# rvl-lab-utoronto/video_similarity_search

Hardware: NVIDIA B200
Metric: finch_full_hierarchy_embeddings_per_s (higher is better)
Workload: dtype f16 screen (f32 accumulate) + f32/f64 exact re-rank

## Files before the change

### video_similarity_search_b200/csrc/nn_screen_tc.cu

```cuda
#include <cuda.h>
#include <cuda_fp16.h>
#include <cuda_fp16.h>
#include <math.h>
#include <stdlib.h>
#include <string.h>
#include <math_constants.h>

#include <algorithm>
#include <type_traits>
#include <vector>

#include "common.cuh"

namespace slic {

constexpr int TC_BM = 128, TC_BK = 64, TC_UMMA_K = 16;
constexpr int TC_BN_WIDE = 256, TC_BN_NARROW = 128;
constexpr int TC_ARES_SPS = 2;
constexpr bool TC_NARROW_ARES = false;
constexpr int TC_ROW_UNIT = 256;
constexpr uint32_t TC_A_BYTES = TC_BM * TC_BK * 2;
constexpr int TC_ARES_MAX_SLABS = 8;
constexpr uint32_t TC_BAR_BYTES = 384;
constexpr int TC_UQ_DEPTH = 4;
constexpr int TC_TMEM_COLS = 512;
template <int NCTA, bool ARES, bool TOPK> struct TcCfg {
    static constexpr int BN = (ARES && TC_NARROW_ARES) ? TC_BN_NARROW : TC_BN_WIDE;
    static constexpr int ACCS = TC_TMEM_COLS / BN;
    static constexpr bool GROUPED = BN == TC_BN_NARROW;
    static constexpr uint32_t B_ROWS = BN / NCTA;
    static constexpr uint32_t B_BYTES = B_ROWS * TC_BK * 2;
    static constexpr uint32_t A_RES_BYTES = ARES ? TC_ARES_MAX_SLABS * TC_A_BYTES : 0;
    static constexpr int SPS = NCTA == 2 ? (ARES ? TC_ARES_SPS : 2) : 1;
    static constexpr uint32_t SLAB_BYTES = ARES ? B_BYTES : TC_A_BYTES + B_BYTES;
    static constexpr uint32_t STAGE_BYTES = SPS * SLAB_BYTES;
    static constexpr int STAGES = ARES ? (TOPK ? 64 : 96) * 1024 / (int)STAGE_BYTES : (NCTA == 1 ? 4 : 3);
    static_assert(STAGES >= 2 && STAGES <= 6, "ring depth");
    static constexpr uint32_t OPERAND_BYTES = A_RES_BYTES + STAGES * STAGE_BYTES;
    static constexpr uint32_t SMEM_BYTES = OPERAND_BYTES + TC_BAR_BYTES  + 960  +
                                           (TOPK ? 32768u : 0u) ;
    static constexpr uint32_t SYM_THR_BYTES = 2 * 2 * 128 * 2;
    static constexpr uint32_t SYM_SMEM_BYTES = OPERAND_BYTES + TC_BAR_BYTES + SYM_THR_BYTES + (ARES ? 640u : 960u);
    static constexpr uint32_t CORESIDENT_MAX_BYTES = 233472 - 2 * 1024;
    static_assert(TOPK || SYM_SMEM_BYTES <= CORESIDENT_MAX_BYTES,
                  "symmetric variant leaves no shared memory for a co-resident CTA of the upload stream");
    static_assert(TOPK || SMEM_BYTES <= CORESIDENT_MAX_BYTES,
                  "top-1 variant (gated launches) leaves no shared memory for a co-resident CTA of the upload stream");
    static_assert(SMEM_BYTES <= 232448, "exceeds the 227 KB of shared memory a CTA may use");
    static_assert(!ARES || NCTA == 2, "the A-resident variant exists for CTA pairs only");
};
constexpr int TC_MAX_STAGES = 6;
constexpr int TC_EPI_WARPS = 8;
constexpr int TC_THREADS = 64 + 32 * TC_EPI_WARPS;
constexpr int TC_THREADS_SYM = TC_THREADS + 32;
constexpr float TC_DEFAULT_EPS = 0.001953125f + 0.0009765625f + 0.0000152587890625f;
constexpr int TC_TOPK_MAX = 64;
constexpr int TC_HIST_BINS = 128;
constexpr int TC_HIST_STRIDE = 2 * TC_BM;
constexpr uint32_t TC_TOPK_SMEM = TC_HIST_BINS * TC_HIST_STRIDE;
static_assert(TC_TOPK_SMEM == 32768, "TcCfg::SMEM_BYTES assumes 32 KB of histograms");

struct ScreenParams {
    int64_t nq, n;
    int num_k_slabs;
    int64_t self_offset;
    float eps;
    int cap;
    int splits;
    int tiles_per_split;
    int64_t num_units;
    int* cand_idx;
    float* cand_score;
    int* cand_cnt;
    int* cand_flags;
    int topk;
    float* cand_kth;
    int* cand_tb;
    int l2_prefetch;
    float* dump;
    int* error_flag;
    unsigned long long* trace;
    const int4* unit_table;
    const int* gates;
    unsigned int* best_enc;
// ... 237 lines not shown
    return u;
}
__device__ __forceinline__ uint32_t cluster_ctarank() {
    uint32_t r;
    asm volatile("mov.u32 %0, %%cluster_ctarank;" : "=r"(r));
    return r;
}
__device__ __forceinline__ void cluster_sync_all() {
    asm volatile("barrier.cluster.arrive.release.aligned;" ::: "memory");
    asm volatile("barrier.cluster.wait.acquire.aligned;" ::: "memory");
}
__device__ __forceinline__ void tc_fence_before() { asm volatile("tcgen05.fence::before_thread_sync;" ::: "memory"); }
__device__ __forceinline__ void tc_fence_after() { asm volatile("tcgen05.fence::after_thread_sync;" ::: "memory"); }
__device__ __forceinline__ void umma_f16(uint32_t tmem_d, uint64_t desc_a, uint64_t desc_b, uint32_t idesc,
                                          uint32_t accumulate) {
    asm volatile(
        "{\n\t.reg .pred p;\n\t"
        "setp.ne.b32 p, %4, 0;\n\t"
        "tcgen05.mma.cta_group::1.kind::f16 [%0], %1, %2, %3, p;\n\t}"
        ::"r"(tmem_d), "l"(desc_a), "l"(desc_b), "r"(idesc), "r"(accumulate)
        : "memory");
}
__device__ __forceinline__ void umma_commit(uint32_t bar) {
    asm volatile("tcgen05.commit.cta_group::1.mbarrier::arrive::one.shared::cluster.b64 [%0];" ::"r"(bar) : "memory");
}
__device__ __forceinline__ void umma_f16_pair(uint32_t tmem_d, uint64_t desc_a, uint64_t desc_b, uint32_t idesc,
                                               uint32_t accumulate) {
    asm volatile(
        "{\n\t.reg .pred p;\n\t"
        "setp.ne.b32 p, %4, 0;\n\t"
        "tcgen05.mma.cta_group::2.kind::f16 [%0], %1, %2, %3, p;\n\t}"
        ::"r"(tmem_d), "l"(desc_a), "l"(desc_b), "r"(idesc), "r"(accumulate)
        : "memory");
}
__device__ __forceinline__ void umma_commit_pair(uint32_t bar) {
    asm volatile(
        "tcgen05.commit.cta_group::2.mbarrier::arrive::one.shared::cluster.multicast::cluster.b64 [%0], %1;"
        ::"r"(bar), "h"((uint16_t)3)
        : "memory");
}
#define SLIC_V32_OUT(v)                                                                                              \
    "=r"(v[0]), "=r"(v[1]), "=r"(v[2]), "=r"(v[3]), "=r"(v[4]), "=r"(v[5]), "=r"(v[6]), "=r"(v[7]), "=r"(v[8]),     \
        "=r"(v[9]), "=r"(v[10]), "=r"(v[11]), "=r"(v[12]), "=r"(v[13]), "=r"(v[14]), "=r"(v[15]), "=r"(v[16]),      \
        "=r"(v[17]), "=r"(v[18]), "=r"(v[19]), "=r"(v[20]), "=r"(v[21]), "=r"(v[22]), "=r"(v[23]), "=r"(v[24]),     \
        "=r"(v[25]), "=r"(v[26]), "=r"(v[27]), "=r"(v[28]), "=r"(v[29]), "=r"(v[30]), "=r"(v[31])
#define SLIC_V32_INOUT(v)                                                                                            \
    "+r"(v[0]), "+r"(v[1]), "+r"(v[2]), "+r"(v[3]), "+r"(v[4]), "+r"(v[5]), "+r"(v[6]), "+r"(v[7]), "+r"(v[8]),     \
        "+r"(v[9]), "+r"(v[10]), "+r"(v[11]), "+r"(v[12]), "+r"(v[13]), "+r"(v[14]), "+r"(v[15]), "+r"(v[16]),      \
        "+r"(v[17]), "+r"(v[18]), "+r"(v[19]), "+r"(v[20]), "+r"(v[21]), "+r"(v[22]), "+r"(v[23]), "+r"(v[24]),     \
        "+r"(v[25]), "+r"(v[26]), "+r"(v[27]), "+r"(v[28]), "+r"(v[29]), "+r"(v[30]), "+r"(v[31])
__device__ __forceinline__ void tmem_ld_issue(uint32_t taddr, uint32_t (&v)[32]) {
    asm volatile(
        "tcgen05.ld.sync.aligned.32x32b.x32.b32 "
        "{%0,%1,%2,%3,%4,%5,%6,%7,%8,%9,%10,%11,%12,%13,%14,%15,%16,%17,%18,%19,%20,%21,%22,%23,%24,%25,%26,%27,%28,"
        "%29,%30,%31}, [%32];"
        : SLIC_V32_OUT(v)
        : "r"(taddr)
        : "memory");
}
__device__ __forceinline__ void tmem_ld_wait(uint32_t (&v)[32]) {
    asm volatile("tcgen05.wait::ld.sync.aligned;" : SLIC_V32_INOUT(v)::"memory");
}

__device__ __forceinline__ uint64_t umma_smem_desc(uint32_t smem_addr) {
    uint64_t d = 0;
    d |= (uint64_t)((smem_addr & 0x3FFFFu) >> 4);
// ... 405 lines not shown
            int stage = 0;
            uint32_t phase = 0, a_phase = 0;
            unsigned long long t_wait = 0;
            const bool scheduler = cta_rank == 0;
            const int stride_groups = (int)(gridDim.x / NCTA);
            auto draw = [&]() -> int { return p.queue_on_peer ? atomicAdd_system(p.queue, 1) : atomicAdd(p.queue, 1); };
            int u_next = scheduler ? (p.queue ? draw() : (int)(blockIdx.x / NCTA)) : 0;
            while (true) {
                int u;
                if (scheduler) {
                    u = u_next < p.num_units ? u_next : -1;
                    mbar_wait_cluster(bar_uq_empty + 8u * ring.slot, ring.phase ^ 1u, p.error_flag);
#pragma unroll
                    for (uint32_t r = 0; r < (uint32_t)NCTA; ++r) {
                        st_cluster_u32(peer_smem_addr(uq_val + 4u * ring.slot, r), (uint32_t)u);
                        mbar_arrive_release_cluster(peer_smem_addr(bar_uq_full + 8u * ring.slot, r));
                    }
                    if (++ring.slot == TC_UQ_DEPTH) {
                        ring.slot = 0;
                        ring.phase ^= 1u;
                    }
                    if (u >= 0) u_next = p.queue ? draw() : u_next + stride_groups;
                } else {
                    u = ring_take(ring, false, p.error_flag);
                }
                if (u < 0) break;
                const UnitInfo ui = unit_info(p, u, n_col_tiles);
                const int64_t row_block = ui.row_unit * NCTA + cta_rank;
                if (ui.gate >= 0) gate_wait(p.gates + ui.gate, p.error_flag);
                if constexpr (SYM) {
                    if (ui.coldir && p.sync_counter)
                        counter_wait(p.sync_counter, __ldg(p.sync_targets + ui.gate + 1), p.error_flag);
                }
                if constexpr (ARES) {
                    mbar_wait_traced(bar_a_empty, a_phase ^ 1, p.error_flag, t_wait, tracing);
                    if (cta_rank == 0) mbar_expect_tx(bar_a_full, 2 * (uint32_t)p.num_k_slabs * TC_A_BYTES);
                    for (int ks = 0; ks < p.num_k_slabs; ++ks)
                        tma_load_2d_pair(&tmap_q, smem_base + ks * TC_A_BYTES, bar_a_full, ks * TC_BK,
                                         (int)(row_block * TC_BM));
                    a_phase ^= 1;
                }
                for (int kt = 0; kt < ui.count; ++kt) {
                    const int64_t ct = ui.ct0 + (int64_t)kt * ui.stride;
                    if (p.l2_prefetch > 0 && kt + p.l2_prefetch < ui.count) {
                        const int64_t ctp = ui.ct0 + (int64_t)(kt + p.l2_prefetch) * ui.stride;
                        for (int ks = 0; ks < p.num_k_slabs; ++ks)
                            tma_prefetch_l2_2d(&tmap_x, ks * TC_BK, (int)(ctp * BN + cta_rank * Cfg::B_ROWS));
                    }
                    for (int ks = 0; ks < p.num_k_slabs; ks += Cfg::SPS) {
                        mbar_wait_traced(bar_empty + 8 * stage, phase ^ 1, p.error_flag, t_wait, tracing);
                        const uint32_t a_dst = ring_base + stage * Cfg::STAGE_BYTES;
                        const uint32_t b_dst = ARES ? a_dst : a_dst + TC_A_BYTES;
                        if constexpr (ARES) {
                            const int nsl = min(Cfg::SPS, p.num_k_slabs - ks);
                            if (cta_rank == 0) mbar_expect_tx(bar_full + 8 * stage, 2 * (uint32_t)nsl * Cfg::B_BYTES);
                            for (int j = 0; j < nsl; ++j)
                                tma_load_2d_pair(&tmap_x, b_dst + j * Cfg::SLAB_BYTES, bar_full + 8 * stage, (ks + j) * TC_BK,
                                                 (int)(ct * BN + cta_rank * Cfg::B_ROWS));
                        } else if constexpr (NCTA == 2) {
                            const int nsl = min(Cfg::SPS, p.num_k_slabs - ks);
                            if (cta_rank == 0) mbar_expect_tx(bar_full + 8 * stage, 2 * (uint32_t)nsl * Cfg::SLAB_BYTES);
                            for (int j = 0; j < nsl; ++j) {
                                tma_load_2d_pair(&tmap_q, a_dst + j * Cfg::SLAB_BYTES, bar_full + 8 * stage, (ks + j) * TC_BK,
                                                 (int)(row_block * TC_BM));
                                tma_load_2d_pair(&tmap_x, b_dst + j * Cfg::SLAB_BYTES, bar_full + 8 * stage, (ks + j) * TC_BK,
                                                 (int)(ct * BN + cta_rank * Cfg::B_ROWS));
                            }
                        } else {
                            mbar_expect_tx(bar_full + 8 * stage, Cfg::STAGE_BYTES);
                            tma_load_2d(&tmap_q, a_dst, bar_full + 8 * stage, ks * TC_BK, (int)(row_block * TC_BM));
                            tma_load_2d(&tmap_x, b_dst, bar_full + 8 * stage, ks * TC_BK, (int)(ct * BN));
                        }
                        if (++stage == STAGES) {
                            stage = 0;
                            phase ^= 1;
                        }
                    }
                }
            }
            if (tracing) atomicAdd(p.trace + 0, t_wait);
        }
    } else if (warp == 1) {
        if (lane == 0 && cta_rank == 0) {
            int stage = 0;
            uint32_t phase = 0;
            int acc = 0;
            uint32_t acc_phase = 0, a_phase = 0;
            unsigned long long t_acc = 0, t_smem = 0;
            const long long t_begin = tracing ? clock64() : 0;
            unsigned long long t_ring = 0, n_units = 0;
            while (true) {
                const long long tr0 = tracing ? clock64() : 0;
                const int u = ring_take(ring, false, p.error_flag);
                if (tracing) t_ring += (unsigned long long)(clock64() - tr0);
                if (u < 0) break;
                ++n_units;
                const int n_tiles = unit_info(p, u, n_col_tiles).count;
                if constexpr (ARES) {
                    mbar_wait_traced(bar_a_full, a_phase, p.error_flag, t_smem, tracing);
                    tc_fence_after();
                    a_phase ^= 1;
                }
                for (int kt = 0; kt < n_tiles; ++kt) {
                    mbar_wait_traced(bar_acc_empty + 8 * acc, acc_phase ^ 1, p.error_flag, t_acc, tracing);
                    tc_fence_after();
                    const uint32_t tmem_d = tmem_base + (uint32_t)(acc * BN);
                    for (int ks = 0; ks < p.num_k_slabs; ks += Cfg::SPS) {
                        mbar_wait_traced(bar_full + 8 * stage, phase, p.error_flag, t_smem, tracing);
                        tc_fence_after();
                        const uint32_t st_addr = ring_base + stage * Cfg::STAGE_BYTES;
#pragma unroll
                        for (int j = 0; j < Cfg::SPS; ++j) {
                            if (ks + j < p.num_k_slabs) {
                                const uint32_t sl_addr = st_addr + j * Cfg::SLAB_BYTES;
                                const uint64_t da = umma_smem_desc(ARES ? smem_base + (ks + j) * TC_A_BYTES : sl_addr);
                                const uint64_t db = umma_smem_desc(ARES ? sl_addr : sl_addr + TC_A_BYTES);
#pragma unroll
                                for (int k = 0; k < TC_BK / TC_UMMA_K; ++k) {
                                    if constexpr (NCTA == 2)
                                        umma_f16_pair(tmem_d, da + (uint64_t)(2 * k), db + (uint64_t)(2 * k), tc_idesc(BN, 2),
                                                       (uint32_t)((ks | j | k) != 0));
                                    else
                                        umma_f16(tmem_d, da + (uint64_t)(2 * k), db + (uint64_t)(2 * k), tc_idesc(BN, 1),
                                                  (uint32_t)((ks | j | k) != 0));
                                }
                            }
                        }
                        if constexpr (NCTA == 2) umma_commit_pair(bar_empty + 8 * stage);
                        else umma_commit(bar_empty + 8 * stage);
                        if (++stage == STAGES) {
                            stage = 0;
                            phase ^= 1;
                        }
                    }
                    if constexpr (NCTA == 2) umma_commit_pair(bar_acc_full + 8 * acc);
                    else umma_commit(bar_acc_full + 8 * acc);
                    if (++acc == ACCS) {
                        acc = 0;
                        acc_phase ^= 1;
                    }
                }
                if constexpr (ARES) umma_commit_pair(bar_a_empty);
            }
            if (tracing) {
                atomicAdd(p.trace + 1, t_acc);
                atomicAdd(p.trace + 2, t_smem);
                atomicAdd(p.trace + 3, (unsigned long long)(clock64() - t_begin));
                atomicAdd(p.trace + 8, t_ring);
                atomicAdd(p.trace + 10, n_units);
            }
        }
    } else if (SYM && warp == 2 + TC_EPI_WARPS) {
        uint16_t* thr_buf = reinterpret_cast<uint16_t*>(smem + Cfg::OPERAND_BYTES + TC_BAR_BYTES);
        constexpr unsigned ENC_POS_INF = 0xff800000u;
        constexpr int PER_LANE = BN / 32;
        constexpr int DIAG_TILES = TC_ROW_UNIT / BN;
        unsigned tile_seq = 0, cseq0 = 0u, cseq1 = 0u;
        for (int u; (u = ring_take(ring, true, p.error_flag)) >= 0;) {
            const UnitInfo ui = unit_info(p, u, n_col_tiles);
            if (!ui.coldir) {
                tile_seq += (unsigned)ui.count;
                continue;
            }
            if (p.sync_counter) {
                if (lane == 0) counter_wait(p.sync_counter, __ldg(p.sync_targets + ui.gate + 1), p.error_flag);
                __syncwarp();
            }
            for (int kt = 0; kt < ui.count; ++kt, ++tile_seq) {
                const int64_t ct = ui.ct0 + (int64_t)kt * ui.stride;
                if (ct / DIAG_TILES == ui.row_unit) continue;
                const int grp = GROUPED ? (int)(tile_seq & 1u) : 0;
                const unsigned cs = grp ? cseq1 : cseq0;
                const uint32_t buf = cs & 1u, ph = (cs >> 1) & 1u;
                const uint32_t bi = (uint32_t)grp * 2u + buf;
                unsigned e[PER_LANE];
#pragma unroll
                for (int j = 0; j < PER_LANE; ++j) {
                    const int64_t c = ct * BN + lane + 32 * j;
                    e[j] = c < p.n ? __ldcg(p.best_enc + c) : ENC_POS_INF;
                }
                mbar_wait(bar_thr_empty + 8 * bi, ph ^ 1u, p.error_flag);
                const uint32_t ta = smem_u32(thr_buf + (GROUPED ? bi * 128u : buf * 256u)) + 2u * lane;
// ... 72 lines not shown
            } else {
                cx.st.best = -CUDART_INF_F;
                cx.st.thr = -CUDART_INF_F;
            }
            cx.st.cnt = 0;
            cx.st.flags = 0;
            uint32_t va[32], vb[32];
            bool prefetched = false;
            bool first = true;
            for (int kt = 0; kt < ui.count; ++kt, ++seq_all) {
                if (GROUPED && (int)(seq_all & 1u) != half) continue;
                const int acc = (int)(seq_all % (unsigned)ACCS);
                const uint32_t acc_phase = (seq_all / (unsigned)ACCS) & 1u;
                const int64_t ct = ui.ct0 + (int64_t)kt * ui.stride;
                const int64_t col0 = GROUPED ? ct * BN : ct * BN + half * 128;
                bool cdir = false;
                uint32_t thr_tile = 0u;
                uint32_t thr_done_bar = 0u;
                if constexpr (SYM) {
                    cdir = ui.coldir && ct / (TC_ROW_UNIT / BN) != ui.row_unit;
                    if (cdir) {
                        const uint32_t buf = tile_seq & 1u, ph = (tile_seq >> 1) & 1u;
                        const uint32_t bi = GROUPED ? (uint32_t)half * 2u + buf : buf;
                        thr_tile = smem_u32(thr_buf + (GROUPED ? bi : buf * 2 + half) * 128);
                        thr_done_bar = bar_thr_empty + 8 * bi;
                        mbar_wait(bar_thr_full + 8 * bi, ph, p.error_flag);
                        ++tile_seq;
                    }
                }
                if (TOPK || !prefetched) {
                    mbar_wait_traced(bar_acc_full + 8 * acc, acc_phase, p.error_flag, t_full, tracing);
                    tc_fence_after();
                }
                const uint32_t tbase = tmem_base + ((uint32_t)(quad * 32) << 16) + (uint32_t)(acc * BN + (GROUPED ? 0 : half * 128));
                if constexpr (TOPK) {
                    cx.count = !first;
                    if (first) {
#pragma unroll 1
                        for (int c = 0; c < 4; ++c) {
                            tmem_ld_issue(tbase + (uint32_t)(c * 32), va);
                            tmem_ld_wait(va);
                            const int64_t col_base = col0 + c * 32;
                            if (col_base >= p.n || !cx.row_ok) continue;
#pragma unroll
                            for (int t = 0; t < 32; ++t) {
                                if (col_base + t < p.n && col_base + t != cx.self_col)
                                    hist_insert(cx.st, cx.hist, __uint_as_float(va[t]), p.topk);
                            }
                            hist_advance(cx.st, cx.hist, p.topk, p.eps);
                        }
                    }
                }
                const bool plain = col0 + 128 <= p.n && !p.dump &&
                                   (p.self_offset < 0 || row_block * TC_BM + p.self_offset + TC_BM <= col0 ||
                                    row_block * TC_BM + p.self_offset >= col0 + 128);
                if constexpr (TOPK) {
                    tmem_ld_issue(tbase, vb);
#pragma unroll 1
                    for (int c = 0; c < 4; ++c) {
                        tmem_ld_wait(vb);
#pragma unroll
                        for (int t = 0; t < 32; ++t) va[t] = vb[t];
                        if (c < 3) {
                            tmem_ld_issue(tbase + (uint32_t)(32 * (c + 1)), vb);
                        } else {
                            tc_fence_before();
                            __syncwarp();
                            if (lane == 0) {
                                if constexpr (NCTA == 2) mbar_arrive_leader(bar_acc_empty + 8 * acc);
                                else mbar_arrive(bar_acc_empty + 8 * acc);
                            }
                        }
                        epi_chunk<TOPK, false>(cx, va, col0 + 32 * c, plain);
                    }
                } else {
                    if (!prefetched) tmem_ld_issue(tbase, va);
                    prefetched = false;
#pragma unroll 1
                    for (int h = 0; h < 2; ++h) {
                        tmem_ld_wait(va);
                        tmem_ld_issue(tbase + (uint32_t)(64 * h + 32), vb);
                        epi_chunk<false, SYM>(cx, va, col0 + 64 * h, plain, cdir, thr_tile + 128u * h);
                        tmem_ld_wait(vb);
                        if (h == 0) {
                            tmem_ld_issue(tbase + 64u, va);
                        } else {
                            tc_fence_before();
                            __syncwarp();
                            if (lane == 0) {
                                if constexpr (NCTA == 2) mbar_arrive_leader(bar_acc_empty + 8 * acc);
                                else mbar_arrive(bar_acc_empty + 8 * acc);
                            }
                            if (kt + (int)TILE_STEP < ui.count) {
                                const unsigned nxt = seq_all + TILE_STEP;
                                const int acc_n = (int)(nxt % (unsigned)ACCS);
                                const bool ready = __all_sync(0xffffffffu, mbar_test(bar_acc_full + 8 * acc_n, (nxt / (unsigned)ACCS) & 1u));
                                if (ready) {
                                    tc_fence_after();
                                    tmem_ld_issue(tmem_base + ((uint32_t)(quad * 32) << 16) +
                                                      (uint32_t)(acc_n * BN + (GROUPED ? 0 : half * 128)), va);
                                    prefetched = true;
                                }
                            }
                        }
                        epi_chunk<false, SYM>(cx, vb, col0 + 64 * h + 32, plain, cdir, thr_tile + 128u * h + 64u);
                    }
                    if constexpr (SYM) {
                        if (cdir) {
                            __syncwarp();
                            if (lane == 0) mbar_arrive(thr_done_bar);
                        }
                    }
                }
                if constexpr (TOPK) {
                    if (first) pend_flush(cx.pd, cx.st, p.eps, p.cap, p.topk, false, cx.hist, cx.li, cx.ls);
                }
                first = false;
            }
            if constexpr (TOPK) pend_flush(cx.pd, cx.st, p.eps, p.cap, p.topk, true, cx.hist, cx.li, cx.ls);
            if constexpr (SYM) {
                if (cx.row_ok && cx.st.best > -CUDART_INF_F) {
                    const unsigned e = enc_score(cx.st.best);
                    atomicMax(p.best_enc + cx.row, e);
                    if (!ui.coldir)
                        for (int g = 0; g < p.num_peers; ++g) atomicMax(p.peer_best[g] + cx.row, e);
                }
                if (!ui.coldir && p.sync_counter) {
                    if (p.num_peers) __threadfence_system();
                    else __threadfence();
                    __syncwarp();
                    if (lane == 0) {
                        atomicAdd(p.sync_counter, 1);
// ... 271 lines not shown
        return SLIC_ERR_CUDA;
    }
    return SLIC_OK;
}

static bool g_profile = false, g_have_sample = false;
static unsigned long long* g_trace = nullptr;
static cudaEvent_t g_ev_start = nullptr, g_ev_stop = nullptr;
static double g_last_flop = 0.0, g_last_exec_flop = 0.0;

struct ScreenPlan {
    int splits, tiles_per_split;
    int64_t units;
};

static int screen_ncta() {
    static int cached = 0;
    if (cached == 0) {
        const char* e = getenv("SLIC_SCREEN_NCTA");
        cached = (e && atoi(e) == 1) ? 1 : 2;
    }
    return cached;
}

static bool screen_ares_allowed() {
    static int cached = -1;
    if (cached < 0) {
        const char* e = getenv("SLIC_SCREEN_ARES");
        cached = (e && atoi(e) == 0) ? 0 : 1;
    }
    return cached != 0;
}

static int screen_bn(int d_pad) {
    return (TC_NARROW_ARES && screen_ncta() == 2 && d_pad / TC_BK <= TC_ARES_MAX_SLABS && screen_ares_allowed()) ? TC_BN_NARROW
                                                                                                                  : TC_BN_WIDE;
}

static ScreenPlan plan_screen(int64_t nq, int64_t n, int bn) {
    const int ncta = screen_ncta();
    const int64_t row_blocks = ceil_div(nq, TC_BM * ncta), col_tiles = ceil_div(n, bn);
    const int64_t sms = num_sms() / ncta;
    int64_t want = ceil_div(6 * sms, row_blocks);
    const int64_t min_tiles = 8 * (TC_BN_WIDE / bn);
    int64_t max_splits = col_tiles / min_tiles > 0 ? col_tiles / min_tiles : 1;
    int64_t splits = want < 1 ? 1 : (want > max_splits ? max_splits : want);
    ScreenPlan pl;
    pl.tiles_per_split = (int)ceil_div(col_tiles, splits);
    pl.splits = (int)ceil_div(col_tiles, pl.tiles_per_split);
    pl.units = row_blocks * pl.splits;
    return pl;
}

static ScreenPlan plan_screen_topk(int64_t nq, int64_t n, int k, int bn) {
    const int ncta = screen_ncta();
    const int64_t row_blocks = ceil_div(nq, TC_BM * ncta), col_tiles = ceil_div(n, bn);
    const int64_t sms = num_sms() / ncta;
    const int64_t startup = 6 * (TC_BN_WIDE / bn);
    int64_t best_s = 1, best_cost = INT64_MAX;
    const int64_t min_tps = ceil_div((int64_t)32 * k, bn / 2);
    for (int pass = 0; pass < 2; ++pass) {
        for (int64_t sp = 1; sp <= col_tiles && sp <= 64; ++sp) {
            const int64_t tps = ceil_div(col_tiles, sp);
            if (sp > 1 && tps < min_tps) break;
            const int64_t real = ceil_div(col_tiles, tps);
            const int64_t waves = ceil_div(row_blocks * real, sms);
            const int64_t cost = waves * (tps + startup);
            if (pass == 0) {
                if (cost < best_cost) {
// ... 43 lines not shown
}

static int* g_timeout_record_host = nullptr;
static int arm_timeout_record() {
    if (!g_timeout_record_host) {
        SLIC_CUDA_OK(cudaHostAlloc(&g_timeout_record_host, 8 * sizeof(int), cudaHostAllocMapped));
        int* dev_view = nullptr;
        SLIC_CUDA_OK(cudaHostGetDevicePointer(&dev_view, g_timeout_record_host, 0));
        SLIC_CUDA_OK(cudaMemcpyToSymbol(g_timeout_record, &dev_view, sizeof(dev_view)));
    }
    for (int i = 0; i < 8; ++i) g_timeout_record_host[i] = 0;
    return SLIC_OK;
}
const char* timeout_record_text() {
    static thread_local char buf[160];
    const int* r = g_timeout_record_host;
    if (!r || r[0] == 0) return "";
    snprintf(buf, sizeof(buf), " [timed-out wait: site %d (1 mbarrier, 2 upload gate, 3 pre-pass counter) block %d thread %d a=%d b=%d]",
             r[0], r[1], r[2], r[3], r[4]);
    return buf;
}

static int launch_screen(const uint16_t* q_f16, int64_t nq, const uint16_t* x_f16, int64_t n, int d_pad,
                         int64_t self_offset, float eps, int cap, const ScreenPlan& pl, int* cand_idx, float* cand_score,
                         int* cand_cnt, int* cand_flags, float* dump, int* error_flag, cudaStream_t st, int topk = 0,
                         float* cand_kth = nullptr, const int4* unit_table = nullptr, const int* gates = nullptr,
                         unsigned int* best_enc = nullptr, int64_t exec_tiles = 0, int* log_q = nullptr,
                         int log_region = 0, int* sync_counter = nullptr, const int* sync_targets = nullptr,
                         const ScreenPeers* peers = nullptr, int* cand_tb = nullptr, int* shared_queue = nullptr) {
    const int ncta = screen_ncta();
    if (gates) SLIC_PROPAGATE(arm_timeout_record());
    CUtensorMap tq, tx;
    SLIC_PROPAGATE(make_tmap(&tq, q_f16, nq, d_pad, TC_BM));
    const int bn = screen_bn(d_pad);
    SLIC_PROPAGATE(make_tmap(&tx, x_f16, n, d_pad, bn / ncta));
    ScreenParams p;
    p.nq = nq;
    p.n = n;
    p.num_k_slabs = d_pad / TC_BK;
    p.self_offset = self_offset;
    p.eps = eps;
    p.cap = cap;
    p.splits = pl.splits;
    p.tiles_per_split = pl.tiles_per_split;
    p.num_units = pl.units;
    p.cand_idx = cand_idx;
    p.cand_score = cand_score;
    p.cand_cnt = cand_cnt;
    p.cand_flags = cand_flags;
    p.topk = topk;
    p.cand_kth = cand_kth;
    p.cand_tb = cand_tb;
    {
        static int l2pf = -1;
        if (l2pf < 0) {
            const char* e = getenv("SLIC_SCREEN_L2PF");
            l2pf = e ? atoi(e) : 0;
            if (l2pf < 0 || l2pf > 16) l2pf = 0;
        }
        p.l2_prefetch = l2pf;
    }
    p.dump = dump;
    p.error_flag = error_flag;
    p.trace = g_trace;
    p.unit_table = unit_table;
    p.gates = gates;
    p.best_enc = best_enc;
// ... 235 lines not shown
                if (need != gate) continue;
                const int64_t ct0 = (int64_t)s * pl->tiles_per_split;
                int64_t cnt = ceil_div(n, bn) - ct0;
                if (cnt > pl->tiles_per_split) cnt = pl->tiles_per_split;
                table->push_back(unit_entry(r, ct0, (int)cnt, 1, gate, s, false));
            }
    SLIC_REQUIRE((int64_t)table->size() == pl->units, "gated screen: internal unit count mismatch");
    return SLIC_OK;
}

template <typename T>
static int nn_top1_sym_impl(const T* unit, const uint16_t* ub, int64_t n, int d, int d_pad, float eps, int* idx_out,
                            T* dist_out, int* stats_out, cudaStream_t st, int part, int parts, const GateSpec* gate,
                            AfterScreenFn after, void* after_ctx, bool* overflowed, int mode = 0,
                            const int* bests_in = nullptr, int* bests_out = nullptr, int* stats_ext = nullptr,
                            const ScreenPeers* peers = nullptr, AfterScreenFn before_screen = nullptr,
                            void* before_ctx = nullptr);
static bool screen_sym_allowed();
constexpr int64_t SYM_MIN_ROWS_FWD = 16384;

template <typename T>
static int nn_top1_impl(const T* q_unit, const uint16_t* q_f16, int64_t nq, const T* x_unit, const uint16_t* x_f16,
                        int64_t n, int d, int d_pad, int64_t self_offset, float eps, int* idx_out, T* dist_out,
                        int* stats_out, cudaStream_t st, const GateSpec* gate = nullptr, AfterScreenFn after = nullptr,
                        void* after_ctx = nullptr, int* stats_ext = nullptr) {
    if (q_f16 == x_f16 && q_unit == x_unit && nq == n && self_offset == 0 && n >= SYM_MIN_ROWS_FWD && screen_sym_allowed()) {
        bool overflowed = false;
        SLIC_PROPAGATE(nn_top1_sym_impl<T>(x_unit, x_f16, n, d, d_pad, eps, idx_out, dist_out, stats_out, st, 0, 1, gate,
                                           after, after_ctx, &overflowed, 0, nullptr, nullptr, stats_ext));
        if (stats_ext || !overflowed) return SLIC_OK;
        gate = nullptr;
        after = nullptr;
    }
    ScreenPlan pl = plan_screen(nq, n, screen_bn(d_pad));
    std::vector<int4> table;
    Scratch table_dev;
    if (gate) {
        SLIC_PROPAGATE(plan_screen_gated(nq, n, screen_bn(d_pad), self_offset, *gate, &pl, &table));
        SLIC_CUDA_OK(table_dev.alloc(table.size() * sizeof(int4), st));
        SLIC_PROPAGATE(stage_to_device(table_dev.ptr, table.data(), table.size() * sizeof(int4), st));
    }
    const int64_t slots = (int64_t)pl.splits * 2 * nq;
    Scratch ci, cs, cc, cf, ovr, stats;
    SLIC_CUDA_OK(ci.alloc(slots * TC_CAP * sizeof(int), st));
    SLIC_CUDA_OK(cs.alloc(slots * TC_CAP * sizeof(float), st));
    SLIC_CUDA_OK(cc.alloc(slots * sizeof(int), st));
    SLIC_CUDA_OK(cf.alloc(slots * sizeof(int), st));
    SLIC_CUDA_OK(ovr.alloc(nq * sizeof(int), st));
    int* stats_dev = stats_ext;
    if (!stats_dev) {
        SLIC_CUDA_OK(stats.alloc(8 * sizeof(int), st));
        stats_dev = stats.as<int>();
    }
    SLIC_CUDA_OK(cudaMemsetAsync(stats_dev, 0, 8 * sizeof(int), st));
    SLIC_PROPAGATE(launch_screen(q_f16, nq, x_f16, n, d_pad, self_offset, eps, TC_CAP, pl, ci.as<int>(), cs.as<float>(),
                                 cc.as<int>(), cf.as<int>(), nullptr, stats_dev + 4, st, 0, nullptr,
                                 gate ? table_dev.as<int4>() : nullptr, gate ? gate->gates : nullptr));
    if (after) SLIC_PROPAGATE(after(after_ctx));
    rerank_top1_kernel<T><<<(unsigned)ceil_div(nq, 8), 256, 0, st>>>(q_unit, x_unit, nq, d, eps, TC_CAP, 2 * pl.splits,
                                                                     ci.as<int>(), cs.as<float>(), cc.as<int>(),
                                                                     cf.as<int>(), idx_out, dist_out, ovr.as<int>(),
                                                                     stats_dev);
    SLIC_LAUNCH_OK();
    if (stats_ext) return SLIC_OK;
    int host_stats[8];
    SLIC_CUDA_OK(cudaMemcpyAsync(host_stats, stats_dev, sizeof(host_stats), cudaMemcpyDeviceToHost, st));
    SLIC_CUDA_OK(cudaStreamSynchronize(st));
    if (host_stats[4] != 0) {
        set_error("nn_screen_kernel: pipeline barrier timed out");
        return SLIC_ERR_CUDA;
    }
    const int n_over = host_stats[1];
    if (n_over > 0) {
        Scratch oi, od;
        SLIC_CUDA_OK(oi.alloc((int64_t)n_over * sizeof(int), st));
        SLIC_CUDA_OK(od.alloc((int64_t)n_over * sizeof(T), st));
        SLIC_PROPAGATE(slic_nn_exact_top1(q_unit, ovr.as<int>(), n_over, x_unit, n, d,
                                          sizeof(T) == 4 ? SLIC_F32 : SLIC_F64, self_offset, oi.as<int>(), od.ptr, st));
        scatter_rows_kernel<T><<<(unsigned)ceil_div(n_over, 256), 256, 0, st>>>(ovr.as<int>(), n_over, oi.as<int>(),
                                                                                od.as<T>(), idx_out, dist_out);
        SLIC_LAUNCH_OK();
    }
    if (stats_out) SLIC_CUDA_OK(cudaMemcpyAsync(stats_out, stats_dev, 4 * sizeof(int), cudaMemcpyDeviceToDevice, st));
    return SLIC_OK;
}

template <typename T>
static int topk_tc_impl(const T* q_unit, const uint16_t* q_f16, int64_t nq, const T* x_unit, const uint16_t* x_f16,
                        int64_t n, int d, int d_pad, int k, int64_t self_offset, float eps, int* idx_out, T* dist_out,
                        int* stats_out, cudaStream_t st) {
    const ScreenPlan pl = plan_screen_topk(nq, n, k, screen_bn(d_pad));
    const int TC_CAP_TOPK = topk_cap(k, (int64_t)pl.tiles_per_split * (screen_bn(d_pad) / 2));
    const int64_t slots = (int64_t)pl.splits * 2 * nq;
    Scratch ci, cs, cc, cf, ck, ctb, ovr, stats;
    SLIC_CUDA_OK(ctb.alloc(slots * sizeof(int), st));
    SLIC_CUDA_OK(cudaMemsetAsync(ctb.ptr, 0, slots * sizeof(int), st));
    SLIC_CUDA_OK(ci.alloc(slots * TC_CAP_TOPK * sizeof(int), st));
    SLIC_CUDA_OK(cs.alloc(slots * TC_CAP_TOPK * sizeof(float), st));
    SLIC_CUDA_OK(cc.alloc(slots * sizeof(int), st));
    SLIC_CUDA_OK(cf.alloc(slots * sizeof(int), st));
    SLIC_CUDA_OK(ck.alloc(slots * sizeof(float), st));
    SLIC_CUDA_OK(ovr.alloc(nq * sizeof(int), st));
    SLIC_CUDA_OK(stats.alloc(8 * sizeof(int), st));
    SLIC_CUDA_OK(cudaMemsetAsync(stats.ptr, 0, 8 * sizeof(int), st));
    SLIC_PROPAGATE(launch_screen(q_f16, nq, x_f16, n, d_pad, self_offset, eps, TC_CAP_TOPK, pl, ci.as<int>(),
                                 cs.as<float>(), cc.as<int>(), cf.as<int>(), nullptr, stats.as<int>() + 4, st, k,
                                 ck.as<float>(), nullptr, nullptr, nullptr, 0, nullptr, 0, nullptr, nullptr, nullptr,
                                 ctb.as<int>()));
    rerank_topk_kernel<T><<<(unsigned)nq, RK_THREADS, 0, st>>>(q_unit, x_unit, nq, d, eps, TC_CAP_TOPK, 2 * pl.splits, k,
                                                               ci.as<int>(), cs.as<float>(), cc.as<int>(), cf.as<int>(),
                                                               ck.as<float>(), idx_out, dist_out, ovr.as<int>(),
                                                               stats.as<int>());
    SLIC_LAUNCH_OK();
    int host_stats[8];
    SLIC_CUDA_OK(cudaMemcpyAsync(host_stats, stats.ptr, sizeof(host_stats), cudaMemcpyDeviceToHost, st));
    SLIC_CUDA_OK(cudaStreamSynchronize(st));
    if (host_stats[4] != 0) {
        set_error("nn_screen_kernel: pipeline barrier timed out");
        return SLIC_ERR_CUDA;
    }
    const int n_over = host_stats[1];
    if (n_over > 0) {
        Scratch oi, od;
        SLIC_CUDA_OK(oi.alloc((int64_t)n_over * k * sizeof(int), st));
        SLIC_CUDA_OK(od.alloc((int64_t)n_over * k * sizeof(T), st));
// ... 113 lines not shown
                                                              const typename DistBits<T>::type* __restrict__ row_min,
                                                              const T* __restrict__ edist, int* __restrict__ idx_out,
                                                              T* __restrict__ dist_out) {
    const int64_t base = (int64_t)blockIdx.x * region;
    const int cnt = log_cnt[blockIdx.x];
    for (int e = threadIdx.x; e < cnt; e += blockDim.x) {
        const T dist = edist[base + e];
        if (dist < (T)0) continue;
        const int q = log_q[base + e];
        if (DistBits<T>::of(dist) == row_min[q]) {
            atomicMin(idx_out + q, log_nb[base + e]);
            if (dist_out) dist_out[q] = dist;
        }
    }
}

__global__ void sym_unsettled_rows_kernel(int* __restrict__ idx_out, int64_t n, int* __restrict__ rows, int* __restrict__ stats) {
    const int64_t i = (int64_t)blockIdx.x * blockDim.x + threadIdx.x;
    if (i < n && idx_out[i] == 0x7fffffff) rows[atomicAdd(&stats[1], 1)] = (int)i;
}

template <typename T>
static int nn_top1_sym_impl(const T* unit, const uint16_t* ub, int64_t n, int d, int d_pad, float eps, int* idx_out,
                            T* dist_out, int* stats_out, cudaStream_t st, int part, int parts, const GateSpec* gate,
                            AfterScreenFn after, void* after_ctx, bool* overflowed, int mode, const int* bests_in,
                            int* bests_out, int* stats_ext, const ScreenPeers* peers, AfterScreenFn before_screen,
                            void* before_ctx) {
    typedef typename DistBits<T>::type Bits;
    *overflowed = false;
    ScreenPlan pl;
    std::vector<int4> table;
    int64_t prepass_units_all = 0;
    const bool shared_list = peers && peers->shared_queue;
    SLIC_PROPAGATE(plan_screen_sym(n, screen_bn(d_pad), part, parts, gate, &pl, &table, (SymMode)mode, &prepass_units_all,
                                   shared_list));
    SLIC_REQUIRE((mode == SYM_FUSED) == (peers != nullptr), "symmetric screen: the fused mode needs peer windows (and only it)");
    SLIC_REQUIRE(mode != SYM_FUSED || (stats_ext && !gate), "symmetric screen: the fused mode is asynchronous and ungated");
    int64_t exec_tiles = 0;
    for (const int4& e : table) exec_tiles += e.z & 0xffff;
    const int num_gates = gate ? gate->num_chunks : 0;
    std::vector<int> targets(num_gates + 1, 0);
    for (const int4& e : table) {
        if ((e.w >> 28) & 1) continue;
        const int g = (e.w & 0xfff) - 1;
        for (int k = g + 1; k <= num_gates; ++k) targets[k] += 2 * TC_EPI_WARPS;
    }
    if (mode == SYM_FUSED) targets[0] = (int)(prepass_units_all * 2 * TC_EPI_WARPS);
    const int64_t groups = num_sms() / 2;
    const int64_t grid = (pl.units < groups ? pl.units : groups) * 2;
    const int64_t regions = grid * TC_EPI_WARPS;
    int64_t capacity = (int64_t)SYM_LOG_PER_ROW * n > SYM_LOG_MIN ? (int64_t)SYM_LOG_PER_ROW * n : SYM_LOG_MIN;
    if (mode == SYM_BESTS) capacity = SYM_LOG_MIN;
    const int64_t region = ceil_div(capacity, regions);
    SLIC_REQUIRE(region < ((int64_t)1 << 31), "symmetric screen: log region too large");
    Scratch table_dev, lq, lnb, ls, lcnt, best, rmin, edist, ovr, stats;
    const size_t table_bytes = table.size() * sizeof(int4);
    SLIC_CUDA_OK(table_dev.alloc(table_bytes + (targets.size() + 4) * sizeof(int), st));
    {
        std::vector<unsigned char> blob(table_bytes + (targets.size() + 1) * sizeof(int));
        memcpy(blob.data(), table.data(), table_bytes);
        const int zero = 0;
        memcpy(blob.data() + table_bytes, &zero, sizeof(int));
        memcpy(blob.data() + table_bytes + sizeof(int), targets.data(), targets.size() * sizeof(int));
        SLIC_PROPAGATE(stage_to_device(table_dev.ptr, blob.data(), blob.size(), st));
    }
    int* sync_dev = reinterpret_cast<int*>(static_cast<unsigned char*>(table_dev.ptr) + table_bytes);
    SLIC_CUDA_OK(lq.alloc(regions * region * sizeof(int), st));
// ... 354 lines not shown
        SLIC_CUDA_OK(cudaDeviceSynchronize());
        SLIC_CUDA_OK(cudaFree(g_trace));
        g_trace = nullptr;
    }
    if (g_trace) SLIC_CUDA_OK(cudaMemset(g_trace, 0, 12 * sizeof(uint64_t)));
    return SLIC_OK;
}

int slic_last_screen_time(float* ms_out, double* flop_out) {
    SLIC_REQUIRE(ms_out && flop_out, "last_screen_time: null pointer");
    if (!slic::g_have_sample) {
        slic::set_error("last_screen_time: no profiled launch (call slic_profile_screen(1) first)");
        return SLIC_ERR_INVALID_ARG;
    }
    SLIC_CUDA_OK(cudaEventSynchronize(slic::g_ev_stop));
    SLIC_CUDA_OK(cudaEventElapsedTime(ms_out, slic::g_ev_start, slic::g_ev_stop));
    *flop_out = slic::g_last_flop;
    return SLIC_OK;
}

int slic_last_screen_exec_flop(double* flop_out) {
    SLIC_REQUIRE(flop_out, "last_screen_exec_flop: null pointer");
    *flop_out = slic::g_have_sample ? slic::g_last_exec_flop : 0.0;
    return SLIC_OK;
}

int slic_screen_scores_debug(const uint16_t* q_f16_dev, int64_t nq, const uint16_t* x_f16_dev, int64_t n,
                             int32_t d_pad, float* out_dev, slic_stream_t stream) {
    using namespace slic;
    SLIC_REQUIRE(nq > 0 && n > 0 && d_pad > 0 && d_pad % 64 == 0, "screen_scores_debug: bad shape");
    SLIC_REQUIRE(q_f16_dev && x_f16_dev && out_dev, "screen_scores_debug: null pointer");
    SLIC_PROPAGATE(slic_require_device());
    cudaStream_t st = as_stream(stream);
    const ScreenPlan pl = plan_screen(nq, n, screen_bn(d_pad));
    const int64_t slots = (int64_t)pl.splits * 2 * nq;
    Scratch ci, cs, cc, cf, err;
    SLIC_CUDA_OK(ci.alloc(slots * TC_CAP * sizeof(int), st));
    SLIC_CUDA_OK(cs.alloc(slots * TC_CAP * sizeof(float), st));
    SLIC_CUDA_OK(cc.alloc(slots * sizeof(int), st));
    SLIC_CUDA_OK(cf.alloc(slots * sizeof(int), st));
    SLIC_CUDA_OK(err.alloc(sizeof(int), st));
    SLIC_CUDA_OK(cudaMemsetAsync(err.ptr, 0, sizeof(int), st));
    SLIC_PROPAGATE(launch_screen(q_f16_dev, nq, x_f16_dev, n, d_pad, -1, TC_DEFAULT_EPS, TC_CAP, pl, ci.as<int>(),
                                 cs.as<float>(), cc.as<int>(), cf.as<int>(), out_dev, err.as<int>(), st));
    int host_err = 0;
    SLIC_CUDA_OK(cudaMemcpyAsync(&host_err, err.ptr, sizeof(int), cudaMemcpyDeviceToHost, st));
    SLIC_CUDA_OK(cudaStreamSynchronize(st));
    if (host_err) {
        set_error("nn_screen_kernel: pipeline barrier timed out");
        return SLIC_ERR_CUDA;
    }
    return SLIC_OK;
}

}
```

Measured before the change: 8.793 million.

## Hold resident query operand in tensor memory for non-top-k A-resident screen

For the A-resident, non-top-k CTA-pair screen, the query slabs are now streamed through the shared-memory ring and copied into tensor memory with tcgen05.cp. The MMAs then take A from TMEM and B from shared memory, using a narrower 128-column tile and two accumulators placed after the A columns. This frees the shared memory that previously held the resident A slabs, which goes to a deeper B ring (6 stages, 4 slabs per stage). The cost is a per-unit TMEM copy step and half-width column tiles, which means more tiles and more epilogue passes.

Result: slower. 7.510 million, median of 6 (-14.6%).

```diff
diff --git a/video_similarity_search_b200/csrc/nn_screen_tc.cu b/video_similarity_search_b200/csrc/nn_screen_tc.cu
--- a/video_similarity_search_b200/csrc/nn_screen_tc.cu
+++ b/video_similarity_search_b200/csrc/nn_screen_tc.cu
@@ -17,30 +17,36 @@
 constexpr int TC_BM = 128, TC_BK = 64, TC_UMMA_K = 16;
 constexpr int TC_BN_WIDE = 256, TC_BN_NARROW = 128;
 constexpr int TC_ARES_SPS = 2;
-constexpr bool TC_NARROW_ARES = false;
 constexpr int TC_ROW_UNIT = 256;
 constexpr uint32_t TC_A_BYTES = TC_BM * TC_BK * 2;
 constexpr int TC_ARES_MAX_SLABS = 8;
 constexpr uint32_t TC_BAR_BYTES = 384;
 constexpr int TC_UQ_DEPTH = 4;
 constexpr int TC_TMEM_COLS = 512;
+constexpr uint32_t TC_TMEM_A_COLS = TC_ARES_MAX_SLABS * TC_BK / 2;
+constexpr int TC_MAX_STAGES = 6;
 template <int NCTA, bool ARES, bool TOPK> struct TcCfg {
-    static constexpr int BN = (ARES && TC_NARROW_ARES) ? TC_BN_NARROW : TC_BN_WIDE;
-    static constexpr int ACCS = TC_TMEM_COLS / BN;
-    static constexpr bool GROUPED = BN == TC_BN_NARROW;
+    static constexpr bool TMEM_A = ARES && !TOPK;
+    static constexpr int BN = TMEM_A ? TC_BN_NARROW : TC_BN_WIDE;
+    static constexpr int ACCS = 2;
+    static constexpr uint32_t ACC_COL0 = TMEM_A ? TC_TMEM_A_COLS : 0u;
+    static_assert(ACC_COL0 + ACCS * BN == TC_TMEM_COLS, "TMEM map");
+    static constexpr bool GROUPED = TMEM_A;
     static constexpr uint32_t B_ROWS = BN / NCTA;
     static constexpr uint32_t B_BYTES = B_ROWS * TC_BK * 2;
-    static constexpr uint32_t A_RES_BYTES = ARES ? TC_ARES_MAX_SLABS * TC_A_BYTES : 0;
-    static constexpr int SPS = NCTA == 2 ? (ARES ? TC_ARES_SPS : 2) : 1;
+    static constexpr uint32_t A_RES_BYTES = (ARES && TOPK) ? TC_ARES_MAX_SLABS * TC_A_BYTES : 0;
+    static constexpr int SPS = TMEM_A ? 4 : NCTA == 2 ? (ARES ? TC_ARES_SPS : 2) : 1;
+    static constexpr int A_SPS = 2;
     static constexpr uint32_t SLAB_BYTES = ARES ? B_BYTES : TC_A_BYTES + B_BYTES;
     static constexpr uint32_t STAGE_BYTES = SPS * SLAB_BYTES;
-    static constexpr int STAGES = ARES ? (TOPK ? 64 : 96) * 1024 / (int)STAGE_BYTES : (NCTA == 1 ? 4 : 3);
-    static_assert(STAGES >= 2 && STAGES <= 6, "ring depth");
+    static_assert(!TMEM_A || A_SPS * TC_A_BYTES == STAGE_BYTES, "an A stage fills a ring stage");
+    static constexpr int STAGES = TMEM_A ? TC_MAX_STAGES : ARES ? 64 * 1024 / (int)STAGE_BYTES : (NCTA == 1 ? 4 : 3);
+    static_assert(STAGES >= 2 && STAGES <= TC_MAX_STAGES, "ring depth");
     static constexpr uint32_t OPERAND_BYTES = A_RES_BYTES + STAGES * STAGE_BYTES;
     static constexpr uint32_t SMEM_BYTES = OPERAND_BYTES + TC_BAR_BYTES  + 960  +
                                            (TOPK ? 32768u : 0u) ;
     static constexpr uint32_t SYM_THR_BYTES = 2 * 2 * 128 * 2;
-    static constexpr uint32_t SYM_SMEM_BYTES = OPERAND_BYTES + TC_BAR_BYTES + SYM_THR_BYTES + (ARES ? 640u : 960u);
+    static constexpr uint32_t SYM_SMEM_BYTES = OPERAND_BYTES + TC_BAR_BYTES + SYM_THR_BYTES + 960u;
     static constexpr uint32_t CORESIDENT_MAX_BYTES = 233472 - 2 * 1024;
     static_assert(TOPK || SYM_SMEM_BYTES <= CORESIDENT_MAX_BYTES,
                   "symmetric variant leaves no shared memory for a co-resident CTA of the upload stream");
@@ -49,7 +55,6 @@
     static_assert(SMEM_BYTES <= 232448, "exceeds the 227 KB of shared memory a CTA may use");
     static_assert(!ARES || NCTA == 2, "the A-resident variant exists for CTA pairs only");
 };
-constexpr int TC_MAX_STAGES = 6;
 constexpr int TC_EPI_WARPS = 8;
 constexpr int TC_THREADS = 64 + 32 * TC_EPI_WARPS;
 constexpr int TC_THREADS_SYM = TC_THREADS + 32;
@@ -353,6 +358,18 @@
         "tcgen05.mma.cta_group::2.kind::f16 [%0], %1, %2, %3, p;\n\t}"
         ::"r"(tmem_d), "l"(desc_a), "l"(desc_b), "r"(idesc), "r"(accumulate)
         : "memory");
+}
+__device__ __forceinline__ void umma_f16_pair_ts(uint32_t tmem_d, uint32_t tmem_a, uint64_t desc_b, uint32_t idesc,
+                                                  uint32_t accumulate) {
+    asm volatile(
+        "{\n\t.reg .pred p;\n\t"
+        "setp.ne.b32 p, %4, 0;\n\t"
+        "tcgen05.mma.cta_group::2.kind::f16 [%0], [%1], %2, %3, p;\n\t}"
+        ::"r"(tmem_d), "r"(tmem_a), "l"(desc_b), "r"(idesc), "r"(accumulate)
+        : "memory");
+}
+__device__ __forceinline__ void tmem_cp_pair(uint32_t taddr, uint64_t desc) {
+    asm volatile("tcgen05.cp.cta_group::2.128x256b [%0], %1;" ::"r"(taddr), "l"(desc) : "memory");
 }
 __device__ __forceinline__ void umma_commit_pair(uint32_t bar) {
     asm volatile(
@@ -824,7 +841,21 @@
                     if (ui.coldir && p.sync_counter)
                         counter_wait(p.sync_counter, __ldg(p.sync_targets + ui.gate + 1), p.error_flag);
                 }
-                if constexpr (ARES) {
+                if constexpr (Cfg::TMEM_A) {
+                    for (int ks = 0; ks < p.num_k_slabs; ks += Cfg::A_SPS) {
+                        mbar_wait_traced(bar_empty + 8 * stage, phase ^ 1, p.error_flag, t_wait, tracing);
+                        const uint32_t dst = ring_base + stage * Cfg::STAGE_BYTES;
+                        const int nsl = min(Cfg::A_SPS, p.num_k_slabs - ks);
+                        if (cta_rank == 0) mbar_expect_tx(bar_full + 8 * stage, 2 * (uint32_t)nsl * TC_A_BYTES);
+                        for (int j = 0; j < nsl; ++j)
+                            tma_load_2d_pair(&tmap_q, dst + j * TC_A_BYTES, bar_full + 8 * stage, (ks + j) * TC_BK,
+                                             (int)(row_block * TC_BM));
+                        if (++stage == STAGES) {
+                            stage = 0;
+                            phase ^= 1;
+                        }
+                    }
+                } else if constexpr (ARES) {
                     mbar_wait_traced(bar_a_empty, a_phase ^ 1, p.error_flag, t_wait, tracing);
                     if (cta_rank == 0) mbar_expect_tx(bar_a_full, 2 * (uint32_t)p.num_k_slabs * TC_A_BYTES);
                     for (int ks = 0; ks < p.num_k_slabs; ++ks)
@@ -880,7 +911,7 @@
             uint32_t acc_phase = 0, a_phase = 0;
             unsigned long long t_acc = 0, t_smem = 0;
             const long long t_begin = tracing ? clock64() : 0;
-            unsigned long long t_ring = 0, n_units = 0;
+            unsigned long long t_ring = 0, n_units = 0, t_head = 0;
             while (true) {
                 const long long tr0 = tracing ? clock64() : 0;
                 const int u = ring_take(ring, false, p.error_flag);
@@ -888,7 +919,31 @@
                 if (u < 0) break;
                 ++n_units;
                 const int n_tiles = unit_info(p, u, n_col_tiles).count;
-                if constexpr (ARES) {
+                if constexpr (Cfg::TMEM_A) {
+                    const long long th0 = tracing ? clock64() : 0;
+                    mbar_wait(bar_a_empty, a_phase ^ 1, p.error_flag);
+                    tc_fence_after();
+                    for (int ks = 0; ks < p.num_k_slabs; ks += Cfg::A_SPS) {
+                        mbar_wait(bar_full + 8 * stage, phase, p.error_flag);
+                        tc_fence_after();
+                        const uint32_t st_addr = ring_base + stage * Cfg::STAGE_BYTES;
+#pragma unroll
+                        for (int j = 0; j < Cfg::A_SPS; ++j) {
+                            if (ks + j < p.num_k_slabs) {
+                                const uint64_t da = umma_smem_desc(st_addr + j * TC_A_BYTES);
+#pragma unroll
+                                for (int k = 0; k < TC_BK / TC_UMMA_K; ++k)
+                                    tmem_cp_pair(tmem_base + (uint32_t)((ks + j) * (TC_BK / 2) + 8 * k), da + (uint64_t)(2 * k));
+                            }
+                        }
+                        umma_commit_pair(bar_empty + 8 * stage);
+                        if (++stage == STAGES) {
+                            stage = 0;
+                            phase ^= 1;
+                        }
+                    }
+                    if (tracing) t_head += (unsigned long long)(clock64() - th0);
+                } else if constexpr (ARES) {
                     mbar_wait_traced(bar_a_full, a_phase, p.error_flag, t_smem, tracing);
                     tc_fence_after();
                     a_phase ^= 1;
@@ -896,7 +951,7 @@
                 for (int kt = 0; kt < n_tiles; ++kt) {
                     mbar_wait_traced(bar_acc_empty + 8 * acc, acc_phase ^ 1, p.error_flag, t_acc, tracing);
                     tc_fence_after();
-                    const uint32_t tmem_d = tmem_base + (uint32_t)(acc * BN);
+                    const uint32_t tmem_d = tmem_base + Cfg::ACC_COL0 + (uint32_t)(acc * BN);
                     for (int ks = 0; ks < p.num_k_slabs; ks += Cfg::SPS) {
                         mbar_wait_traced(bar_full + 8 * stage, phase, p.error_flag, t_smem, tracing);
                         tc_fence_after();
@@ -909,7 +964,10 @@
                                 const uint64_t db = umma_smem_desc(ARES ? sl_addr : sl_addr + TC_A_BYTES);
 #pragma unroll
                                 for (int k = 0; k < TC_BK / TC_UMMA_K; ++k) {
-                                    if constexpr (NCTA == 2)
+                                    if constexpr (Cfg::TMEM_A)
+                                        umma_f16_pair_ts(tmem_d, tmem_base + (uint32_t)((ks + j) * (TC_BK / 2) + 8 * k),
+                                                         db + (uint64_t)(2 * k), tc_idesc(BN, 2), (uint32_t)((ks | j | k) != 0));
+                                    else if constexpr (NCTA == 2)
                                         umma_f16_pair(tmem_d, da + (uint64_t)(2 * k), db + (uint64_t)(2 * k), tc_idesc(BN, 2),
                                                        (uint32_t)((ks | j | k) != 0));
                                     else
@@ -933,6 +991,7 @@
                     }
                 }
                 if constexpr (ARES) umma_commit_pair(bar_a_empty);
+                if constexpr (Cfg::TMEM_A) a_phase ^= 1;
             }
             if (tracing) {
                 atomicAdd(p.trace + 1, t_acc);
@@ -940,6 +999,7 @@
                 atomicAdd(p.trace + 3, (unsigned long long)(clock64() - t_begin));
                 atomicAdd(p.trace + 8, t_ring);
                 atomicAdd(p.trace + 10, n_units);
+                atomicAdd(p.trace + 11, t_head);
             }
         }
     } else if (SYM && warp == 2 + TC_EPI_WARPS) {
@@ -1078,7 +1138,8 @@
                     mbar_wait_traced(bar_acc_full + 8 * acc, acc_phase, p.error_flag, t_full, tracing);
                     tc_fence_after();
                 }
-                const uint32_t tbase = tmem_base + ((uint32_t)(quad * 32) << 16) + (uint32_t)(acc * BN + (GROUPED ? 0 : half * 128));
+                const uint32_t tbase = tmem_base + ((uint32_t)(quad * 32) << 16) + Cfg::ACC_COL0 +
+                                       (uint32_t)(acc * BN + (GROUPED ? 0 : half * 128));
                 if constexpr (TOPK) {
                     cx.count = !first;
                     if (first) {
@@ -1143,7 +1204,7 @@
                                 const bool ready = __all_sync(0xffffffffu, mbar_test(bar_acc_full + 8 * acc_n, (nxt / (unsigned)ACCS) & 1u));
                                 if (ready) {
                                     tc_fence_after();
-                                    tmem_ld_issue(tmem_base + ((uint32_t)(quad * 32) << 16) +
+                                    tmem_ld_issue(tmem_base + ((uint32_t)(quad * 32) << 16) + Cfg::ACC_COL0 +
                                                       (uint32_t)(acc_n * BN + (GROUPED ? 0 : half * 128)), va);
                                     prefetched = true;
                                 }
@@ -1481,9 +1542,9 @@
     return cached != 0;
 }
 
-static int screen_bn(int d_pad) {
-    return (TC_NARROW_ARES && screen_ncta() == 2 && d_pad / TC_BK <= TC_ARES_MAX_SLABS && screen_ares_allowed()) ? TC_BN_NARROW
-                                                                                                                  : TC_BN_WIDE;
+static int screen_bn(int d_pad, bool topk) {
+    return (!topk && screen_ncta() == 2 && d_pad / TC_BK <= TC_ARES_MAX_SLABS && screen_ares_allowed()) ? TC_BN_NARROW
+                                                                                                        : TC_BN_WIDE;
 }
 
 static ScreenPlan plan_screen(int64_t nq, int64_t n, int bn) {
@@ -1593,7 +1654,7 @@
     if (gates) SLIC_PROPAGATE(arm_timeout_record());
     CUtensorMap tq, tx;
     SLIC_PROPAGATE(make_tmap(&tq, q_f16, nq, d_pad, TC_BM));
-    const int bn = screen_bn(d_pad);
+    const int bn = screen_bn(d_pad, topk > 0);
     SLIC_PROPAGATE(make_tmap(&tx, x_f16, n, d_pad, bn / ncta));
     ScreenParams p;
     p.nq = nq;
@@ -1895,11 +1956,11 @@
         gate = nullptr;
         after = nullptr;
     }
-    ScreenPlan pl = plan_screen(nq, n, screen_bn(d_pad));
+    ScreenPlan pl = plan_screen(nq, n, screen_bn(d_pad, false));
     std::vector<int4> table;
     Scratch table_dev;
     if (gate) {
-        SLIC_PROPAGATE(plan_screen_gated(nq, n, screen_bn(d_pad), self_offset, *gate, &pl, &table));
+        SLIC_PROPAGATE(plan_screen_gated(nq, n, screen_bn(d_pad, false), self_offset, *gate, &pl, &table));
         SLIC_CUDA_OK(table_dev.alloc(table.size() * sizeof(int4), st));
         SLIC_PROPAGATE(stage_to_device(table_dev.ptr, table.data(), table.size() * sizeof(int4), st));
     }
@@ -1952,8 +2013,8 @@
 static int topk_tc_impl(const T* q_unit, const uint16_t* q_f16, int64_t nq, const T* x_unit, const uint16_t* x_f16,
                         int64_t n, int d, int d_pad, int k, int64_t self_offset, float eps, int* idx_out, T* dist_out,
                         int* stats_out, cudaStream_t st) {
-    const ScreenPlan pl = plan_screen_topk(nq, n, k, screen_bn(d_pad));
-    const int TC_CAP_TOPK = topk_cap(k, (int64_t)pl.tiles_per_split * (screen_bn(d_pad) / 2));
+    const ScreenPlan pl = plan_screen_topk(nq, n, k, screen_bn(d_pad, true));
+    const int TC_CAP_TOPK = topk_cap(k, (int64_t)pl.tiles_per_split * (screen_bn(d_pad, true) / 2));
     const int64_t slots = (int64_t)pl.splits * 2 * nq;
     Scratch ci, cs, cc, cf, ck, ctb, ovr, stats;
     SLIC_CUDA_OK(ctb.alloc(slots * sizeof(int), st));
@@ -2133,7 +2194,7 @@
     std::vector<int4> table;
     int64_t prepass_units_all = 0;
     const bool shared_list = peers && peers->shared_queue;
-    SLIC_PROPAGATE(plan_screen_sym(n, screen_bn(d_pad), part, parts, gate, &pl, &table, (SymMode)mode, &prepass_units_all,
+    SLIC_PROPAGATE(plan_screen_sym(n, screen_bn(d_pad, false), part, parts, gate, &pl, &table, (SymMode)mode, &prepass_units_all,
                                    shared_list));
     SLIC_REQUIRE((mode == SYM_FUSED) == (peers != nullptr), "symmetric screen: the fused mode needs peer windows (and only it)");
     SLIC_REQUIRE(mode != SYM_FUSED || (stats_ext && !gate), "symmetric screen: the fused mode is asynchronous and ungated");
@@ -2554,7 +2615,7 @@
     SLIC_REQUIRE(q_f16_dev && x_f16_dev && out_dev, "screen_scores_debug: null pointer");
     SLIC_PROPAGATE(slic_require_device());
     cudaStream_t st = as_stream(stream);
-    const ScreenPlan pl = plan_screen(nq, n, screen_bn(d_pad));
+    const ScreenPlan pl = plan_screen(nq, n, screen_bn(d_pad, false));
     const int64_t slots = (int64_t)pl.splits * 2 * nq;
     Scratch ci, cs, cc, cf, err;
     SLIC_CUDA_OK(ci.alloc(slots * TC_CAP * sizeof(int), st));
```
